# ittiam-systems/libxaac

Hardware: AMD Instinct MI355X
Metric: decoded audio frames/s (1024-spl IMDCT + complex QMF + HQ SBR + parametric stereo, HE-AACv2) (higher is better)
Workload: dtype int32

## Files before the change

### libxaac_amd/csrc/sbr_ps_frame.h

```cpp
#ifndef XAAC_SBR_PS_FRAME_H
#define XAAC_SBR_PS_FRAME_H

#include <stddef.h>

#include "sbr_ps.h"

#ifndef XP_T
#define XP_T(i)
#endif

#define XP_NO_PS_SCALE 0x7fffffff
#define XP_MAX_SEG (XAAC_PS_MAX_ENV + 2)

#if defined(__HIPCC__)
#define XP_UNROLL _Pragma("unroll")
#define XP_NOUNROLL _Pragma("nounroll")
#define XP_LAMBDA_INLINE __attribute__((always_inline))
#else
#define XP_UNROLL
#define XP_NOUNROLL
#define XP_LAMBDA_INLINE
#endif

struct XpFrameWork {
  union {
    int32_t hyb_u[3][2][44];
    uint32_t gscan[32][8];
    int32_t peak[32][20];
    uint32_t dl[32][13];
  };
  int32_t hyb_l[32][20];
  union {
    int32_t binpw[32][20];
    int16_t ratio[32][20];
  };
  uint32_t ap_h[32][11];
  uint32_t seg_hd[XP_MAX_SEG][4][24];
};
template <bool B>
struct XpBool {
  static constexpr bool value = B;
};

FX_HD int xp_popc(uint32_t v) { return __builtin_popcount(v); }
FX_HD int xp_clz(uint32_t v) { return __builtin_clz(v); }
FX_HD uint32_t xp_pack16(int16_t lo, int16_t hi) { return (uint32_t)(uint16_t)lo | ((uint32_t)(uint16_t)hi << 16); }
FX_HD int16_t xp_lo16(uint32_t v) { return (int16_t)(v & 0xffffu); }
FX_HD int16_t xp_hi16(uint32_t v) { return (int16_t)(v >> 16); }

FX_HD int32_t xp_dot2(uint32_t a, uint32_t b) {
#if defined(__HIP_DEVICE_COMPILE__)
  int32_t r;
  asm("v_dot2_i32_i16 %0, %1, %2, 0" : "=v"(r) : "v"(a), "v"(b));
  return r;
#else
  return (int32_t)((uint32_t)((int32_t)xp_lo16(a) * xp_lo16(b)) + (uint32_t)((int32_t)xp_hi16(a) * xp_hi16(b)));
#endif
}
FX_HD int16_t xp_seg_coeff(uint32_t hd, int n) { return (int16_t)(xp_hi16(hd) + n * xp_lo16(hd)); }
FX_HD uint32_t xp_load_pair(const int16_t *p) {
#if defined(__HIP_DEVICE_COMPILE__)
  typedef uint32_t __attribute__((may_alias)) xp_u32_alias;
  return *reinterpret_cast<const xp_u32_alias *>(p);
#else
  return xp_pack16(p[0], p[1]);
#endif
}
struct XpPhase {
  uint32_t re_pair, im_pair;
};
FX_HD XpPhase xp_phase_pairs(int16_t re, int16_t im) {
  XpPhase p;
  p.re_pair = xp_pack16(re, (int16_t)-im);
  p.im_pair = xp_pack16(im, re);
  return p;
}
FX_HD uint32_t xp_q15_pair(int32_t a, int32_t b) {
  return (((uint32_t)a >> 15) & 0xffffu) | (((uint32_t)b << 1) & 0xffff0000u);
}
FX_HD uint32_t xp_hi_pair(int32_t a, int32_t b) {
#if defined(__HIP_DEVICE_COMPILE__)
  return __builtin_amdgcn_perm((uint32_t)b, (uint32_t)a, 0x07060302u);
#else
  return ((uint32_t)a >> 16) | ((uint32_t)b & 0xffff0000u);
#endif
}
FX_HD uint32_t xp_mult16_shl_pair(uint32_t p, int32_t f2) {
#if defined(__HIP_DEVICE_COMPILE__)
  return xp_hi_pair(__mul24(xp_lo16(p), f2), __mul24(xp_hi16(p), f2));
#else
  return xp_hi_pair((int32_t)((uint32_t)(int32_t)xp_lo16(p) * (uint32_t)f2), (int32_t)((uint32_t)(int32_t)xp_hi16(p) * (uint32_t)f2));
#endif
}
FX_HD int32_t xp_m16x16_shl_pre(int16_t a, int32_t b2) {
#if defined(__HIP_DEVICE_COMPILE__)
  return __mul24(a, b2);
#else
  return (int32_t)((uint32_t)(int32_t)a * (uint32_t)b2);
#endif
}
FX_HD uint32_t xp_add16_pair(uint32_t a, uint32_t b) {
#if defined(__HIP_DEVICE_COMPILE__)
  typedef short xp_short2 __attribute__((ext_vector_type(2)));
  return __builtin_bit_cast(uint32_t, (xp_short2)(__builtin_bit_cast(xp_short2, a) + __builtin_bit_cast(xp_short2, b)));
#else
  return ((a + b) & 0xffffu) | ((a & 0xffff0000u) + (b & 0xffff0000u));
#endif
}
FX_HD uint32_t xp_sub16_pair(uint32_t a, uint32_t b) {
#if defined(__HIP_DEVICE_COMPILE__)
  typedef short xp_short2 __attribute__((ext_vector_type(2)));
  return __builtin_bit_cast(uint32_t, (xp_short2)(__builtin_bit_cast(xp_short2, a) - __builtin_bit_cast(xp_short2, b)));
#else
  return ((a - b) & 0xffffu) | ((a & 0xffff0000u) - (b & 0xffff0000u));
#endif
}
FX_HD uint32_t xp_allpass_packed(uint32_t &d0, uint32_t new_pair, const XpPhase &ph, uint32_t &e0, uint32_t &e1, uint32_t &e2,
                                 const XpPhase &p0, const XpPhase &p1, const XpPhase &p2, int16_t decay0, int16_t decay1,
                                 int16_t decay2) {
  uint32_t in = xp_q15_pair(xp_dot2(d0, ph.re_pair), xp_dot2(d0, ph.im_pair));
  d0 = new_pair;
  uint32_t *e[3] = {&e0, &e1, &e2};
  const XpPhase *pp[3] = {&p0, &p1, &p2};
  const int32_t decay2x[3] = {2 * decay0, 2 * decay1, 2 * decay2};
  XP_UNROLL
  for (int m = 0; m < 3; m++) {
    const uint32_t s = *e[m];
    const uint32_t t = xp_sub16_pair(xp_q15_pair(xp_dot2(s, pp[m]->re_pair), xp_dot2(s, pp[m]->im_pair)),
                                     xp_mult16_shl_pair(in, decay2x[m]));
    *e[m] = xp_add16_pair(in, xp_mult16_shl_pair(t, decay2x[m]));
    in = t;
  }
  return in;
}

FX_HD int32_t xp_adj_word(int32_t v, int shift) {
  if (shift > 31) shift = 31;
  if (shift < -31) shift = -31;
  const int shl = shift > 0 ? shift : 0, shr = shift < 0 ? -shift : 0;
  return (int32_t)((uint32_t)v << shl) >> shr;
}

FX_HD int32_t xp_bin_power_hyb(const XpTables *T, int bin, const int32_t *re, const int32_t *im) {
  if (bin < 2) {
    const int a = bin == 0 ? 0 : 4, b = bin == 0 ? 5 : 1;
    int32_t pw = xp_power(re[a], im[a]);
    pw = fx_add_sat(pw, fx_mul32x16(re[b], (int16_t)(re[b] >> 16)));
    return fx_add_sat(pw, fx_mul32x16(im[b], (int16_t)(im[b] >> 16)));
  }
  const int sb = T->borders_group[bin + 2];
  return xp_power(re[sb], im[sb]);
}

FX_HD uint32_t xp_gsum_addend(int32_t pw, int group_shift, bool counts) { return counts ? (uint32_t)(pw >> group_shift) : 0u; }
FX_HD uint32_t xp_gsum_scan(const XsCx &cx, uint32_t a, uint32_t &run) {
#if defined(__HIP_DEVICE_COMPILE__)
  int32_t r = (int32_t)a;
#define XP_DPP_ADD(ctrl, rows) r += __builtin_amdgcn_update_dpp(0, r, ctrl, rows, 0xf, false);
  XP_DPP_ADD(0x111, 0xf)
  XP_DPP_ADD(0x112, 0xf)
  XP_DPP_ADD(0x114, 0xf)
  XP_DPP_ADD(0x118, 0xf)
  XP_DPP_ADD(0x142, 0xa)
  XP_DPP_ADD(0x143, 0xc)
#undef XP_DPP_ADD
  (void)cx;
  (void)run;
  return (uint32_t)r;
#else
  (void)cx;
  run += a;
  return run;
#endif
}
FX_HD int32_t xp_gsum_sum(uint32_t s_last, uint32_t s_before) {
  const uint32_t d = s_last - s_before;
  return (int32_t)(d < 0x7fffffffu ? d : 0x7fffffffu);
}
FX_HD bool xp_gsum_fits(const XpTables *T) {
  if (T->borders_group[16] != 9) return false;
  for (int g = 0; g < 6; g++) {
    const int b0 = T->borders_group[16 + g], b1 = T->borders_group[17 + g], shift = T->group_shift[g];
    if (b1 <= b0 || b1 > 64 || shift < 0 || shift > 31) return false;
    if ((uint64_t)(b1 - b0) * (uint64_t)(0x7fffffff >> shift) >= ((uint64_t)1 << 32)) return false;
  }
  return true;
}

template <int NS = 32, class PS>
FX_HD int xp_ps_frame(const XsCx &cx, const XpTables *T, PS *ps, const xaac_ps_frame *pf, XpFrameWork *w, int32_t *xl,
                      int32_t *xr, int lb_scale, int ov_lb_scale, int hb_scale, int st_syn, int lsb, int usb,
                      int ps_scale_done = XP_NO_PS_SCALE) {
  static_assert(NS == 32 || NS == 30, "frames of 32 or 30 QMF slots");
#if defined(__HIP_DEVICE_COMPILE__)
  int32_t p1v[3][2], p3re[32], p3im[32];
  {
    const int l1 = cx.lane & 31;
    XP_UNROLL
    for (int b = 0; b < 3; b++) {
      p1v[b][0] = xl[(l1 + 6) * 128 + b];
      p1v[b][1] = xl[(l1 + 6) * 128 + 64 + b];
    }
    XP_UNROLL
    for (int l = 0; l < 32; l++) {
      p3re[l] = NS == 32 || l < NS ? xl[l * 128 + cx.lane] : 0;
      p3im[l] = NS == 32 || l < NS ? xl[l * 128 + 64 + cx.lane] : 0;
    }
  }
#endif
  const int ps_scale = ps_scale_done != XP_NO_PS_SCALE ? ps_scale_done : xp_init_ps_scale(cx, ps, lb_scale, ov_lb_scale, hb_scale);
  const int ov_lb_shift = ps_scale - ov_lb_scale, lb_shift = ps_scale - lb_scale, hb_shift = ps_scale - hb_scale;
  const int common_shift = (st_syn - ps_scale) - 8;
  XP_T(1);

  XS_PAR(l, 0, NS) {
    const int shiftdelay = l < NS - 6 ? 0 : (int16_t)(lb_scale - ps_scale);
    for (int b = 0; b < 3; b++) {
      const int sha = l + 6 < NS ? (b < lsb ? lb_shift : (b < usb ? hb_shift : 0)) : 0;
      for (int c = 0; c < 2; c++) {
#if defined(__HIP_DEVICE_COMPILE__)
        int32_t v = xp_adj_word(p1v[b][c], sha);
#else
        int32_t v = xp_adj_word(xl[(l + 6) * 128 + 64 * c + b], sha);
#endif
        v = shiftdelay < 0 ? fx_shl(v, -shiftdelay) : fx_shr(v, shiftdelay);
        w->hyb_u[b][c][12 + l] = v;
      }
    }
  }
  XS_PAR(i, 0, 12)
    for (int b = 0; b < 3; b++) {
      w->hyb_u[b][0][i] = ps->hyb_buf[b][0][i];
      w->hyb_u[b][1][i] = ps->hyb_buf[b][1][i];
    }
  cx.sync();
  XS_PAR(l, 0, NS) {
    int32_t re[8], im[8];
    xp_filt_8ch(T, &w->hyb_u[0][0][l], &w->hyb_u[0][1][l], re, im);
    for (int k = 0; k < 6; k++) {
      w->hyb_l[l][k] = re[k];
      w->hyb_l[l][10 + k] = im[k];
    }
  }
  XS_PAR(i, 0, 64) {
    const int b = 1 + (i >> 5), l = i & 31;
    if (NS != 32 && l >= NS) continue;
    int32_t re[2], im[2];
    xp_filt_2ch(T, &w->hyb_u[b][0][l], &w->hyb_u[b][1][l], re, im);
    w->hyb_l[l][4 + 2 * b] = re[0];
    w->hyb_l[l][5 + 2 * b] = re[1];
    w->hyb_l[l][14 + 2 * b] = im[0];
    w->hyb_l[l][15 + 2 * b] = im[1];
  }
  XS_PAR(i, 0, 12)
    for (int b = 0; b < 3; b++) {
      ps->hyb_buf[b][0][i] = w->hyb_u[b][0][NS + i];
      ps->hyb_buf[b][1][i] = w->hyb_u[b][1][NS + i];
    }
  cx.sync();
  XP_T(2);

  XS_PAR(g, 0, XAAC_PS_GROUPS) {
    w->seg_hd[0][0][g] = xp_pack16(ps->delta_h11_h12[2 * g], ps->H11_H12[2 * g]);
    w->seg_hd[0][1][g] = xp_pack16(ps->delta_h11_h12[2 * g + 1], ps->H11_H12[2 * g + 1]);
    w->seg_hd[0][2][g] = xp_pack16(ps->delta_h21_h22[2 * g], ps->H21_H22[2 * g]);
    w->seg_hd[0][3][g] = xp_pack16(ps->delta_h21_h22[2 * g + 1], ps->H21_H22[2 * g + 1]);
  }
  const int usb_prev = cx.uni(ps->usb);
  uint32_t seg_mask = 0;
  int clear_slot = NS;
  {
    int env = 0, nseg = 1;
    int next = cx.uni(pf->border_position[0]);
    for (int l = 0; l < NS; l++) {
      if (l == next) {
        if (env == 0) clear_slot = l;
        cx.sync();
        xp_rot_env_coeffs(cx, T, ps, pf, env);
        XS_PAR(g, 0, XAAC_PS_GROUPS) {
          w->seg_hd[nseg][0][g] = xp_pack16(ps->delta_h11_h12[2 * g], ps->H11_H12[2 * g]);
          w->seg_hd[nseg][1][g] = xp_pack16(ps->delta_h11_h12[2 * g + 1], ps->H11_H12[2 * g + 1]);
          w->seg_hd[nseg][2][g] = xp_pack16(ps->delta_h21_h22[2 * g], ps->H21_H22[2 * g]);
          w->seg_hd[nseg][3][g] = xp_pack16(ps->delta_h21_h22[2 * g + 1], ps->H21_H22[2 * g + 1]);
        }
        seg_mask |= 1u << l;
        nseg++;
        env++;
        next = env <= XAAC_PS_MAX_ENV ? cx.uni(pf->border_position[env]) : 64;
      }
    }
  }
  cx.sync();
  XP_T(3);

  {
    XP_UNROLL
    for (int c = 0; c < 4; c++) {
      uint32_t run[8] = {0, 0, 0, 0, 0, 0, 0, 0};
      XS_PAR(sb, 0, 64) {
        int32_t rre[8], rim[8];
        XP_UNROLL
        for (int ls = 0; ls < 8; ls++) {
#if defined(__HIP_DEVICE_COMPILE__)
          rre[ls] = p3re[8 * c + ls];
          rim[ls] = p3im[8 * c + ls];
#else
          rre[ls] = xl[(8 * c + ls) * 128 + sb];
          rim[ls] = xl[(8 * c + ls) * 128 + 64 + sb];
#endif
        }
        const int gsh = sb < 11 ? 0 : (sb < 18 ? 1 : (sb < 23 ? 2 : (sb < 35 ? 3 : 4)));
        const bool own_bin = sb >= 3 && sb < 9;
        int gcol = 6;
        XP_UNROLL
        for (int g = 0; g < 6; g++) gcol = sb == T->borders_group[17 + g] - 1 ? g : gcol;
        int32_t *dst = own_bin ? &w->binpw[8 * c][sb + 5] : reinterpret_cast<int32_t *>(&w->gscan[8 * c][gcol]);
        const int dstride = own_bin ? 20 : 8;
        XP_UNROLL
        for (int ls = 0; ls < 8; ls++) {
          const int l = 8 * c + ls;
          const int usb_l = l >= clear_slot ? usb : usb_prev;
          const int sh = sb < lsb ? (l < 6 ? ov_lb_shift : lb_shift) : (sb < usb ? hb_shift : 0);
          const int32_t re = xp_adj_word(rre[ls], sh), im = xp_adj_word(rim[ls], sh);
          const int32_t pw = xp_power(re, im);
          const uint32_t s = xp_gsum_scan(cx, xp_gsum_addend(pw, gsh, sb >= 9 && sb < usb_l), run[ls]);
          dst[ls * dstride] = own_bin ? pw : (int32_t)s;
        }
      }
    }
  }
  cx.sync();
  XS_PAR(i, 0, 6 * NS) {
    const int l = i / 6, g = i % 6;
    const uint32_t prev = w->gscan[l][g > 0 ? g - 1 : 0];
    const uint32_t before = g > 0 ? prev : 0u;
    w->binpw[l][14 + g] = xp_gsum_sum(w->gscan[l][g], before);
  }
  XS_PAR(i, 0, 8 * NS) {
    const int l = i >> 3, bin = i & 7;
    w->binpw[l][bin] = xp_bin_power_hyb(T, bin, &w->hyb_l[l][0], &w->hyb_l[l][10]);
  }
  cx.sync();
  XP_T(4);

  XS_PAR(bin, 0, 20) {
    int32_t pd = ps->peak_decay_diff[bin], pdp = ps->peak_decay_diff_prev[bin], nrg = ps->energy_prev[bin];
    int32_t pin[NS];
    XP_UNROLL
    for (int l = 0; l < NS; l++) pin[l] = w->binpw[l][bin];
    XP_UNROLL
    for (int l = 0; l < NS; l++) {
      int32_t pw = fx_shl(pin[l], 1);
      if (pw < 0) pw = 0;
      pd = fx_mul32x16_shl(pd, 0x620a);
      if (pw > pd) pd = pw;
      pdp = fx_add_sat(fx_mul32x16_shl(pdp, 0x6000), fx_sub_sat(pd, pw) >> 2);
      nrg = fx_add_sat(fx_mul32x16_shl(nrg, 0x6000), pw >> 2);
      w->binpw[l][bin] = nrg;
      w->peak[l][bin] = fx_add_sat(pdp, pdp >> 1);
    }
    ps->peak_decay_diff[bin] = pd;
    ps->peak_decay_diff_prev[bin] = pdp;
    ps->energy_prev[bin] = nrg;
  }
  cx.sync();
  for (int i0 = 0; i0 < 20 * NS; i0 += 64) {
    int16_t q = 0;
    XS_PAR(i, i0, (20 * NS) % 64 == 0 || i0 + 64 < 20 * NS ? i0 + 64 : 20 * NS) {
      const int32_t pk = (&w->peak[0][0])[i], nrg = (&w->binpw[0][0])[i];
      q = pk <= nrg ? (int16_t)0x7fff : (int16_t)xp_divide16_pos(nrg, pk);
#if !defined(__HIP_DEVICE_COMPILE__)
      (&w->ratio[0][0])[i] = q;
#endif
    }
#if defined(__HIP_DEVICE_COMPILE__)
    cx.sync();
    (&w->ratio[0][0])[i0 + cx.lane] = q;
    cx.sync();
#endif
  }
  cx.sync();
  XP_T(5);

  {
    const int idx0 = cx.uni(ps->idx), idx_long0 = cx.uni(ps->idx_long);
    const int is0 = cx.uni(ps->idx_ser[0]), is1 = cx.uni(ps->idx_ser[1]), is2 = cx.uni(ps->idx_ser[2]);
    const int clear_lo = (usb > usb_prev && usb_prev) ? usb_prev : 64;
    const int clear_hi = usb < 23 ? usb : 23;
    const int p14_0 = idx_long0 % 14;
    const int cs_right = common_shift < 0 ? (-common_shift > 31 ? 31 : -common_shift) : 0;
    uint32_t events = seg_mask | (1u << 6) | (1u << 14);
    if (clear_slot < NS) events |= 1u << clear_slot;
    if (clear_slot + 14 < NS) events |= 1u << (clear_slot + 14);
    XS_PAR(sb, 0, 64) {
      const int qmf_chain = sb >= 3 && sb < 23, hyb_chain = sb >= 32 && sb < 42, chain = qmf_chain || hyb_chain;
      const int csb = qmf_chain ? sb : (hyb_chain ? sb - 32 : 3);
      const int di = 9 + 3 * (csb - 3);
      const int16_t *ph = hyb_chain ? &T->frac_delay_phase_fac_qmf_sub_re_im[2 * csb] : &T->frac_delay_phase_fac_qmf_re_im[2 * csb];
      const int16_t *pser = hyb_chain ? &T->frac_delay_phase_fac_qmf_sub_ser_re_im[2 * csb] : &T->frac_delay_phase_fac_qmf_ser_re_im[2 * csb];
      const int pstep = hyb_chain ? 32 : 64;
      const XpPhase phase = xp_phase_pairs(ph[0], ph[1]);
      const XpPhase ps0 = xp_phase_pairs(pser[0], pser[1]), ps1 = xp_phase_pairs(pser[pstep], pser[pstep + 1]),
                    ps2 = xp_phase_pairs(pser[2 * pstep], pser[2 * pstep + 1]);
      const int16_t dec0 = hyb_chain ? T->rev_link_decay_ser[0] : T->decay_scale_factor[qmf_chain ? di : 9];
      const int16_t dec1 = hyb_chain ? T->rev_link_decay_ser[1] : T->decay_scale_factor[qmf_chain ? di + 1 : 10];
      const int16_t dec2 = hyb_chain ? T->rev_link_decay_ser[2] : T->decay_scale_factor[qmf_chain ? di + 2 : 11];
      uint32_t d0[2] = {0, 0}, r0[3] = {0, 0, 0}, r1[4] = {0, 0, 0, 0}, r2[5] = {0, 0, 0, 0, 0};
      if (chain) {
        XP_UNROLL
        for (int j = 0; j < 2; j++) {
          const int16_t *q = hyb_chain ? &ps->sub[(idx0 + j) % 2][2 * csb] : &ps->ap[(idx0 + j) % 2][2 * csb];
          d0[j] = xp_pack16(q[0], q[1]);
        }
        XP_UNROLL
        for (int j = 0; j < 3; j++) {
          const int16_t *q = hyb_chain ? &ps->sub_ser[(is0 + j) % 3][0][2 * csb] : &ps->ser[(is0 + j) % 3][0][2 * csb];
          r0[j] = xp_pack16(q[0], q[1]);
        }
        XP_UNROLL
        for (int j = 0; j < 4; j++) {
          const int16_t *q = hyb_chain ? &ps->sub_ser[(is1 + j) % 4][1][2 * csb] : &ps->ser[(is1 + j) % 4][1][2 * csb];
          r1[j] = xp_pack16(q[0], q[1]);
        }
        XP_UNROLL
        for (int j = 0; j < 5; j++) {
          const int16_t *q = hyb_chain ? &ps->sub_ser[(is2 + j) % 5][2][2 * csb] : &ps->ser[(is2 + j) % 5][2][2 * csb];
          r2[j] = xp_pack16(q[0], q[1]);
        }
      }
      const int g = T->band_to_group[sb];
      const int bin_sb = sb < 23 ? T->delay_to_bin[sb] : (sb < 35 ? 18 : 19);
      uint32_t h11, h12, h21, h22, d11, d12, d21, d22;
      const auto seg_load = [&](int s) {
        const uint32_t a = w->seg_hd[s][0][g], b = w->seg_hd[s][1][g], c = w->seg_hd[s][2][g], d = w->seg_hd[s][3][g];
        h11 = a & 0xffff0000u, h12 = b & 0xffff0000u, h21 = c & 0xffff0000u, h22 = d & 0xffff0000u;
        d11 = a << 16, d12 = b << 16, d21 = c << 16, d22 = d << 16;
      };
      seg_load(0);
      uint32_t prev = sb >= 35 ? xp_pack16(ps->sd[2 * (sb - 35)], ps->sd[2 * (sb - 35) + 1]) : 0u;
      const int is_ap = sb < 23, is_d14 = sb >= 23 && sb < 35;
      int shl_ov, shr_ov, shl_lb, shr_lb;
      {
        const int s_ov = sb < lsb ? ov_lb_shift : (sb < usb ? hb_shift : 0), s_lb = sb < lsb ? lb_shift : (sb < usb ? hb_shift : 0);
        const int c_ov = s_ov > 31 ? 31 : (s_ov < -31 ? -31 : s_ov), c_lb = s_lb > 31 ? 31 : (s_lb < -31 ? -31 : s_lb);
        shl_ov = c_ov > 0 ? c_ov : 0, shr_ov = c_ov < 0 ? -c_ov : 0;
        shl_lb = c_lb > 0 ? c_lb : 0, shr_lb = c_lb < 0 ? -c_lb : 0;
      }
      int shl = shl_ov, shr = shr_ov;
      bool active = sb < usb_prev, fed14 = false;
      const int ldj = is_d14 ? 2 * (sb - 23) : 0, dlj = is_d14 ? sb - 23 : 12, apj = hyb_chain ? csb : 10;
      int ld_at = 24 * p14_0;
      const int16_t *const ld_lane = &ps->ld[0][ldj];
      static_assert(sizeof(ps->ld[0]) == 24 * sizeof(int16_t), "rows of the 14-slot ring: 24 int16, whole words");
      static_assert(offsetof(PS, ld) % 4 == 0 && alignof(PS) % 4 == 0, "the 14-slot ring starts on a word of a word-aligned state");
      int16_t tr_nx = w->ratio[0][bin_sb];
      int32_t hre_nx = w->hyb_l[0][csb], him_nx = w->hyb_l[0][10 + csb];
      uint32_t ld_nx = xp_load_pair(ld_lane + ld_at);
      int32_t nre[4], nim[4];
      XP_UNROLL
      for (int j = 0; j < 4; j++) {
        nre[j] = xl[j * 128 + sb];
        nim[j] = xl[j * 128 + 64 + sb];
      }
      const auto walk = [&](auto cs_positive) XP_LAMBDA_INLINE {
        XP_NOUNROLL
        for (int l0 = 0; l0 < NS; l0 += 4) {
          int32_t cre[4], cim[4];
          XP_UNROLL
          for (int j = 0; j < 4; j++) {
            cre[j] = nre[j];
            cim[j] = nim[j];
          }
          if (l0 + 4 < NS) {
            XP_UNROLL
            for (int j = 0; j < 4; j++) {
              nre[j] = xl[(l0 + 4 + j) * 128 + sb];
              nim[j] = xl[(l0 + 4 + j) * 128 + 64 + sb];
            }
          }
          const uint32_t events4 = events >> l0;
          XP_UNROLL
          for (int j = 0; j < 4; j++) {
            const int l = l0 + j;
            if (NS % 4 != 0 && l >= NS) break;
            const int16_t tr = tr_nx;
            const int32_t hre = hre_nx, him = him_nx;
            const uint32_t ld_cur = ld_nx;
            {
              const int ln = l + 1 < NS ? l + 1 : NS - 1;
              ld_at = ld_at + 24 == 14 * 24 ? 0 : ld_at + 24;
              tr_nx = w->ratio[ln][bin_sb];
              hre_nx = w->hyb_l[ln][csb];
              him_nx = w->hyb_l[ln][10 + csb];
              ld_nx = xp_load_pair(ld_lane + ld_at);
            }
            if ((events4 >> j) & 1u) {
#if defined(__HIP_DEVICE_COMPILE__)
              asm volatile("");
#endif
              shl = l < 6 ? shl_ov : shl_lb;
              shr = l < 6 ? shr_ov : shr_lb;
              active = sb < (l >= clear_slot ? usb : usb_prev);
              fed14 = l >= 14 && sb < (l - 14 >= clear_slot ? usb : usb_prev);
              if (l == clear_slot) {
                const int c = qmf_chain && sb >= clear_lo && sb < clear_hi;
                XP_UNROLL
                for (int m = 0; m < 3; m++) r0[m] = c ? 0u : r0[m];
                XP_UNROLL
                for (int m = 0; m < 4; m++) r1[m] = c ? 0u : r1[m];
                XP_UNROLL
                for (int m = 0; m < 5; m++) r2[m] = c ? 0u : r2[m];
              }
              if ((seg_mask >> l) & 1u)
                seg_load(xp_popc(seg_mask & (0xffffffffu >> (31 - l))));
            }
            const int32_t re0 = (int32_t)((uint32_t)cre[j] << shl) >> shr, im0 = (int32_t)((uint32_t)cim[j] << shl) >> shr;
            const int16_t q_re = fx_round16(re0), q_im = fx_round16(im0);
            const uint32_t q = xp_pack16(q_re, q_im);
            const uint32_t in_pair = hyb_chain ? xp_pack16(fx_round16(hre), fx_round16(him)) : q;
            uint32_t dv = d0[0], e0 = r0[0], e1 = r1[0], e2 = r2[0];
            const uint32_t o_chain = xp_allpass_packed(dv, in_pair, phase, e0, e1, e2, ps0, ps1, ps2, dec0, dec1, dec2);
            d0[0] = d0[1];
            d0[1] = dv;
            r0[0] = r0[1]; r0[1] = r0[2];
            r0[2] = e0;
            r1[0] = r1[1]; r1[1] = r1[2]; r1[2] = r1[3];
            r1[3] = e1;
            r2[0] = r2[1]; r2[1] = r2[2]; r2[2] = r2[3]; r2[3] = r2[4];
            r2[4] = e2;
            w->ap_h[l][apj] = o_chain;
            h11 += d11;
            h12 += d12;
            h21 += d21;
            h22 += d22;
            const uint32_t o14_new = w->dl[l >= 14 ? l - 14 : 0][dlj];
            const uint32_t o14 = fed14 ? o14_new : ld_cur;
            const uint32_t o = is_ap ? o_chain : (is_d14 ? o14 : prev);
            w->dl[l][dlj] = q;
            prev = active ? q : prev;
            int32_t re = re0, im = im0;
            int32_t r_re = xp_m16x16_shl_pre(xp_lo16(o), 2 * tr), r_im = xp_m16x16_shl_pre(xp_hi16(o), 2 * tr);
            xp_rotate_w(&re, &r_re, h11, h12, h21, h22);
            xp_rotate_w(&im, &r_im, h11, h12, h21, h22);
            re = active ? re : re0;
            im = active ? im : im0;
            r_re = active ? r_re : 0;
            r_im = active ? r_im : 0;
            if (decltype(cs_positive)::value) {
              re = fx_shl_sat(re, common_shift);
              im = fx_shl_sat(im, common_shift);
            } else {
              re = re >> cs_right;
              im = im >> cs_right;
            }
            if (sb >= 3) {
              xl[l * 128 + sb] = re;
              xl[l * 128 + 64 + sb] = im;
              xr[l * 128 + sb] = r_re;
              xr[l * 128 + 64 + sb] = r_im;
            }
          }
        }
      };
      if (common_shift > 0)
        walk(XpBool<true>());
      else
        walk(XpBool<false>());
      if (chain) {
        XP_UNROLL
        for (int j = 0; j < 2; j++) {
          int16_t *q = hyb_chain ? &ps->sub[(idx0 + j) % 2][2 * csb] : &ps->ap[(idx0 + j) % 2][2 * csb];
          q[0] = xp_lo16(d0[j]);
          q[1] = xp_hi16(d0[j]);
        }
        XP_UNROLL
        for (int j = 0; j < 3; j++) {
          int16_t *q = hyb_chain ? &ps->sub_ser[(is0 + NS + j) % 3][0][2 * csb] : &ps->ser[(is0 + NS + j) % 3][0][2 * csb];
          q[0] = xp_lo16(r0[j]);
          q[1] = xp_hi16(r0[j]);
        }
        XP_UNROLL
        for (int j = 0; j < 4; j++) {
          int16_t *q = hyb_chain ? &ps->sub_ser[(is1 + NS + j) % 4][1][2 * csb] : &ps->ser[(is1 + NS + j) % 4][1][2 * csb];
          q[0] = xp_lo16(r1[j]);
          q[1] = xp_hi16(r1[j]);
        }
        XP_UNROLL
        for (int j = 0; j < 5; j++) {
          int16_t *q = hyb_chain ? &ps->sub_ser[(is2 + NS + j) % 5][2][2 * csb] : &ps->ser[(is2 + NS + j) % 5][2][2 * csb];
          q[0] = xp_lo16(r2[j]);
          q[1] = xp_hi16(r2[j]);
        }
      }
      if (sb >= 35) {
        ps->sd[2 * (sb - 35)] = xp_lo16(prev);
        ps->sd[2 * (sb - 35) + 1] = xp_hi16(prev);
      }
      if (is_d14) {
        for (int l = (clear_slot == 0 || usb == usb_prev) ? NS - 14 : 0; l < NS; l++) {
          const int pos = (idx_long0 + l) % 14;
          if (sb < (l >= clear_slot ? usb : usb_prev)) {
            ps->ld[pos][ldj] = xp_lo16(w->dl[l][dlj]);
            ps->ld[pos][ldj + 1] = xp_hi16(w->dl[l][dlj]);
          }
        }
      }
    }
    cx.sync();
    XS_ONE {
      ps->idx = (int16_t)idx0;
      ps->idx_ser[0] = (int16_t)((is0 + NS) % 3);
      ps->idx_ser[1] = (int16_t)((is1 + NS) % 4);
      ps->idx_ser[2] = (int16_t)((is2 + NS) % 5);
      ps->idx_long = (int16_t)((idx_long0 + NS) % 14);
      if (clear_slot < NS) ps->usb = (int16_t)usb;
    }
  }
  cx.sync();
  XP_T(6);

  XS_PAR(i, 0, 2 * NS) {
    const int l = i >> 1, c = i & 1;
    const uint32_t below = seg_mask & (0xffffffffu >> (31 - l));
    const int s = xp_popc(below), nn = l - (below ? 31 - xp_clz(below) : 0) + 1;
    int32_t acc_l[3] = {0, 0, 0}, acc_r[3] = {0, 0, 0};
    XP_UNROLL
    for (int sb = 0; sb < 10; sb++) {
      const int b = sb < 6 ? 0 : (sb < 8 ? 1 : 2);
      const bool first = sb == 0 || sb == 6 || sb == 8;
      const int16_t h11 = xp_seg_coeff(w->seg_hd[s][0][sb], nn), h12 = xp_seg_coeff(w->seg_hd[s][1][sb], nn);
      const int16_t h21 = xp_seg_coeff(w->seg_hd[s][2][sb], nn), h22 = xp_seg_coeff(w->seg_hd[s][3][sb], nn);
      const int16_t tr = w->ratio[l][T->hybrid_to_bin[sb]];
      const uint32_t o = w->ap_h[l][sb];
      int32_t lv = w->hyb_l[l][10 * c + sb];
      int32_t rv = xp_m16x16_shl(c ? xp_hi16(o) : xp_lo16(o), tr);
      xp_rotate(&lv, &rv, h11, h12, h21, h22);
      acc_l[b] = first ? lv : fx_add_sat(acc_l[b], lv);
      acc_r[b] = first ? rv : fx_add_sat(acc_r[b], rv);
    }
    XP_UNROLL
    for (int b = 0; b < 3; b++) {
      int32_t v = acc_l[b];
      if (common_shift < 0)
        v = fx_shr(v, -common_shift > 31 ? 31 : -common_shift);
      else if (common_shift > 0)
        v = fx_shl_sat(v, common_shift);
      xl[l * 128 + 64 * c + b] = v;
      xr[l * 128 + 64 * c + b] = acc_r[b];
    }
  }
  {
    const int s = xp_popc(seg_mask), n = NS - (seg_mask ? 31 - xp_clz(seg_mask) : 0);
    XS_PAR(g, 0, XAAC_PS_GROUPS) {
      ps->H11_H12[2 * g] = xp_seg_coeff(w->seg_hd[s][0][g], n);
      ps->H11_H12[2 * g + 1] = xp_seg_coeff(w->seg_hd[s][1][g], n);
      ps->H21_H22[2 * g] = xp_seg_coeff(w->seg_hd[s][2][g], n);
      ps->H21_H22[2 * g + 1] = xp_seg_coeff(w->seg_hd[s][3][g], n);
    }
  }
  cx.sync();
  XP_T(7);
  return ps_scale;
}

#endif
```

### libxaac_amd/csrc/sbr_ps_kernel.hip

```cpp
#include <hip/hip_runtime.h>
#include <stddef.h>
#include <stdint.h>
#include <stdlib.h>

#ifdef XS_PROFILE
__shared__ long long xp_prof_last;
__shared__ long long xp_prof_acc[16];
#define XP_T(i)                                   \
  do {                                            \
    if (threadIdx.x == 0) {                       \
      long long t_ = clock64();                   \
      xp_prof_acc[i] += t_ - xp_prof_last;        \
      xp_prof_last = t_;                          \
    }                                             \
  } while (0)
#else
#define XP_T(i)
#endif
#define XS_SYNC_WAVE_LDS 1
#include "sbr_ps_frame.h"
#include "sbr_ps_kernel.h"

namespace {

struct XpLdsState {
  XAAC_PS_STATE_HEAD_FIELDS
};
constexpr int kHeadWords = offsetof(xaac_ps_state, syn_ring_r) / 4;
static_assert(offsetof(xaac_ps_state, syn_ring_r) % 4 == 0 && sizeof(XpLdsState) == kHeadWords * 4, "mirror layout");
static_assert(sizeof(xaac_ps_frame) % 4 == 0, "word copies");

constexpr int kTabBytes = (int)sizeof(XpTables);
#ifndef XP_WAVES
#define XP_WAVES 4
#endif
#ifndef XP_WAVES_PER_EU
#define XP_WAVES_PER_EU 2
#endif
constexpr int kPsWaves = XP_WAVES;
struct XpLds {
  XpLdsState ps;
  xaac_ps_frame pf;
  XpFrameWork w;
};

__device__ __forceinline__ void xp_wave_sync() {
  __builtin_amdgcn_fence(__ATOMIC_RELEASE, "wavefront");
  __builtin_amdgcn_wave_barrier();
  __builtin_amdgcn_fence(__ATOMIC_ACQUIRE, "wavefront");
}

__device__ __forceinline__ void copy_words(int32_t *dst, const int32_t *src, int n, int lane) {
  for (int i = lane; i < n; i += 64 * 8) {
    int32_t t[8];
#pragma unroll
    for (int j = 0; j < 8; j++)
      if (i + 64 * j < n) t[j] = src[i + 64 * j];
#pragma unroll
    for (int j = 0; j < 8; j++)
      if (i + 64 * j < n) dst[i + 64 * j] = t[j];
  }
}

template <int NS>
__device__ __forceinline__ int xp_init_ps_scale_regs(const XsCx &cx, int32_t (&rs)[NS], int lb_scale, int ov_lb_scale, int hb_scale) {
  constexpr int W_AP = offsetof(XpLdsState, ap) / 4, W_LD = offsetof(XpLdsState, ld) / 4, W_SD = offsetof(XpLdsState, sd) / 4;
  constexpr int W_SUB = offsetof(XpLdsState, sub) / 4, W_IDX = offsetof(XpLdsState, idx_ser) / 4;
  constexpr int W_PK = offsetof(XpLdsState, peak_decay_diff) / 4, W_HYB = offsetof(XpLdsState, hyb_buf) / 4;
  constexpr int W_H = offsetof(XpLdsState, h11_h12_vec) / 4, W_DBS = offsetof(XpLdsState, delay_buffer_scale) / 4;
  static_assert(offsetof(XpLdsState, ser) == 0 && W_AP == 480 && W_LD == W_AP + 64 && W_SD == W_LD + 168 && W_SUB == W_SD + 32, "layout");
  static_assert(W_IDX == W_SUB + 32 + 240 && offsetof(XpLdsState, sample_ser) == 4 * W_IDX + 6 && W_PK == W_IDX + 4, "layout");
  static_assert(W_HYB == W_PK + 60 && W_H == W_HYB + 72 && offsetof(XpLdsState, delay_buffer_scale) % 4 == 0 && W_DBS < 64 * NS, "layout");
  const auto word_of = [&](int w) { return __builtin_amdgcn_readlane(rs[w / 64], w % 64); };
  const int ss0 = word_of(W_IDX + 1) >> 16, ss1 = (int16_t)word_of(W_IDX + 2), ss2 = word_of(W_IDX + 2) >> 16;
  const auto is_pair = [&](int w) -> bool {
    const int k = w & 31, blk = w >> 5;
    const bool mid = k >= 3 && k <= 22;
    if (w < W_AP) {
      const int i = blk % 3, j = blk / 3;
      return mid && j < (i == 0 ? ss0 : (i == 1 ? ss1 : ss2));
    }
    if (w < W_LD) return mid;
    if (w < W_SD + 29) return true;
    if (w < W_SUB) return false;
    return w < W_IDX;
  };
  int32_t m16 = 0, m32 = 0;
#pragma unroll
  for (int j = 0; j < NS; j++) {
    const int w = cx.lane + 64 * j;
    const int32_t v = rs[j], lo = (int16_t)v, hi = v >> 16;
    m16 |= is_pair(w) ? (fx_abs_nrm(lo) | fx_abs_nrm(hi)) : 0;
    if (64 * j + 63 >= W_HYB && 64 * j < W_H) m32 |= (w >= W_HYB && w < W_H) ? fx_abs_nrm(v) : 0;
  }
  const int reserve = xs_pnorm32(cx.wave_or((int32_t)((uint32_t)m16 << 16) | m32));
  const int dbs = (int16_t)((int16_t)word_of(W_DBS) + reserve);
  int16_t t = (int16_t)(lb_scale < ov_lb_scale ? lb_scale : ov_lb_scale);
  if (hb_scale < t) t = (int16_t)hb_scale;
  if (dbs < t) t = (int16_t)dbs;
  const int ps_scale = t - 1;
  const int scale = (int16_t)((ps_scale - dbs) + reserve);
  if (scale != 0) {
    const int l16 = scale > 0 ? (scale > 15 ? 15 : scale) : 0, r16 = scale < 0 ? (-scale > 31 ? 31 : -scale) : 0;
#pragma unroll
    for (int j = 0; j < NS; j++) {
      const int w = cx.lane + 64 * j;
      const int32_t v = rs[j];
      if (64 * j < W_IDX) {
        const int32_t lo = (int16_t)v, hi = v >> 16;
        const int16_t a = fx_sat16(xs_shl(lo, l16) >> r16), b = fx_sat16(xs_shl(hi, l16) >> r16);
        rs[j] = is_pair(w) ? (int32_t)xp_pack16(a, b) : v;
      }
      if (64 * j + 63 >= W_PK && 64 * j < W_H) {
        const bool pk = w >= W_PK && w < W_HYB, hy = w >= W_HYB && w < W_H;
        const int sc = pk ? 2 * scale : scale;
        const int32_t r = sc > 0 ? fx_shl_sat(rs[j], sc) : fx_shr(rs[j], -sc);
        rs[j] = (pk || hy) ? r : rs[j];
      }
    }
  }
  if (cx.lane == W_DBS % 64) rs[W_DBS / 64] = (int32_t)((uint32_t)rs[W_DBS / 64] & 0xffff0000u) | (uint16_t)(int16_t)ps_scale;
  return ps_scale;
}

template <int NF, int NSL = 32>
__device__ __forceinline__ int xp_frame_sanitize_regs(const XsCx &cx, int32_t (&rf)[NF]) {
  constexpr int E_BORDER = offsetof(xaac_ps_frame, border_position) / 2, E_IID = offsetof(xaac_ps_frame, iid_par_table) / 2;
  constexpr int E_ICC = offsetof(xaac_ps_frame, icc_par_table) / 2, E_END = sizeof(xaac_ps_frame) / 2;
  static_assert(offsetof(xaac_ps_frame, iid_quant) == 0 && E_BORDER + XAAC_PS_MAX_ENV + 2 < E_IID && E_IID % 2 == 0 && E_ICC % 2 == 0, "layout");
  const int steps = (int16_t)__builtin_amdgcn_readlane(rf[0], 0) ? 15 : 7;
  int bad = 0;
#pragma unroll
  for (int j = 0; j < NF; j++) {
    const int w = cx.lane + 64 * j;
    const int32_t v = rf[j];
    int h[2] = {(int16_t)v, v >> 16};
#pragma unroll
    for (int c = 0; c < 2; c++) {
      const int e = 2 * w + c;
      const bool border = e >= E_BORDER && e < E_BORDER + XAAC_PS_MAX_ENV + 2, iid = e >= E_IID && e < E_ICC, icc = e >= E_ICC && e < E_END;
      const int lo = border ? 0 : (iid ? -steps : (icc ? 0 : -32768)), hi = border ? NSL : (iid ? steps : (icc ? 7 : 32767));
      const int t = h[c] < lo ? lo : (h[c] > hi ? hi : h[c]);
      bad |= t != h[c];
      h[c] = t;
    }
    rf[j] = (int32_t)xp_pack16((int16_t)h[0], (int16_t)h[1]);
  }
  return cx.wave_or(bad) != 0;
}

}

template <int NSL = 32>
__global__ __launch_bounds__(64 * kPsWaves, XP_WAVES_PER_EU) void xaac_ps_kernel(XaacPsParams p) {
  __shared__ XpLds sw[kPsWaves];
  __shared__ int32_t s_tabs[(kTabBytes + 3) / 4];
  const int lane = threadIdx.x & 63, wave = __builtin_amdgcn_readfirstlane(threadIdx.x >> 6);
  XpLds &s = sw[wave];
  const XsCx cx = {lane, 64};
  for (int i = threadIdx.x; i < (kTabBytes + 3) / 4; i += 64 * kPsWaves) s_tabs[i] = reinterpret_cast<const int32_t *>(&xaac_ps_tables)[i];
  __syncthreads();
  const XpTables *tabs = reinterpret_cast<const XpTables *>(s_tabs);
#ifdef XP_STAGGER_G
  if (p.n >= 3 * (int)gridDim.x * kPsWaves)
    for (int t = 0; t < ((int)blockIdx.x * kPsWaves + wave) % XP_STAGGER_G; t++) __builtin_amdgcn_s_sleep(XP_STAGGER_SLEEP);
#endif
#ifdef XS_PROFILE
  if (threadIdx.x == 0) {
    for (int i = 0; i < 16; i++) xp_prof_acc[i] = 0;
  }
#endif
  for (int n = blockIdx.x * kPsWaves + wave; n < p.n; n += gridDim.x * kPsWaves) {
    xaac_ps_state *gps = p.state + n;
    int32_t *gx = p.x + (size_t)n * (40 * 128) + 2 * 128;
    int32_t *gr = p.xr + (size_t)n * (32 * 128);
    int16_t *par = p.par_l + 8 * (size_t)n;
    constexpr int NS = (kHeadWords + 63) / 64, NF = (sizeof(xaac_ps_frame) / 4 + 63) / 64;
    int32_t rs[NS], rf[NF];
    const int32_t *gs = reinterpret_cast<const int32_t *>(gps), *gf = reinterpret_cast<const int32_t *>(p.frame + n);
    const int apply_v = p.sbr_frame[n].apply_processing, mode_v = p.header[n].channel_mode;
    const int par_v = lane < (NSL != 32 ? 8 : 6) ? par[lane] : 0;
    const int tail_v = lane < 3 ? (lane == 0 ? gps->st_syn_scale_r : (lane == 1 ? gps->syn_lsb_r : gps->syn_usb_r)) : 0;

#pragma unroll
    for (int j = 0; j < NS; j++) rs[j] = lane + 64 * j < kHeadWords ? gs[lane + 64 * j] : 0;
#pragma unroll
    for (int j = 0; j < NF; j++) rf[j] = lane + 64 * j < (int)(sizeof(xaac_ps_frame) / 4) ? gf[lane + 64 * j] : 0;
    if (NSL != 32 && __builtin_amdgcn_readlane(par_v, 7)) {
      if (lane == 0) p.par_r[8 * (size_t)n + 6] = 1;
      continue;
    }
    if (!(__builtin_amdgcn_readfirstlane(apply_v) && __builtin_amdgcn_readfirstlane(mode_v) == 3)) {
      if (lane == 0) {
        p.par_l[8 * (size_t)n + 6] = 0;
        p.par_r[8 * (size_t)n + 6] = 1;
      }
      continue;
    }
    const int lb_scale = __builtin_amdgcn_readlane(par_v, 0), ov_lb_scale = __builtin_amdgcn_readlane(par_v, 1);
    const int hb_scale = __builtin_amdgcn_readlane(par_v, 2), st_syn = __builtin_amdgcn_readlane(par_v, 3);
    const int lsb = __builtin_amdgcn_readlane(par_v, 4), usb = __builtin_amdgcn_readlane(par_v, 5);
    const int ps_scale_done = xp_init_ps_scale_regs<NS>(cx, rs, lb_scale, ov_lb_scale, hb_scale);
    const int ps_clamped = xp_frame_sanitize_regs<NF, NSL>(cx, rf);
    xp_wave_sync();
#pragma unroll
    for (int j = 0; j < NS; j++)
      if (lane + 64 * j < kHeadWords) reinterpret_cast<int32_t *>(&s.ps)[lane + 64 * j] = rs[j];
#pragma unroll
    for (int j = 0; j < NF; j++)
      if (lane + 64 * j < (int)(sizeof(xaac_ps_frame) / 4)) reinterpret_cast<int32_t *>(&s.pf)[lane + 64 * j] = rf[j];
    xp_wave_sync();
#ifdef XS_PROFILE
    if (threadIdx.x == 0) xp_prof_last = clock64();
#endif
    const int ps_scale =
        xp_ps_frame<NSL>(cx, tabs, &s.ps, &s.pf, &s.w, gx, gr, lb_scale, ov_lb_scale, hb_scale, st_syn, lsb, usb, ps_scale_done);
    xp_wave_sync();
    {
      int32_t *dst = reinterpret_cast<int32_t *>(gps);
      const int32_t *src = reinterpret_cast<const int32_t *>(&s.ps);
      for (int i = lane; i < kHeadWords; i += 64) dst[i] = src[i];
    }
    if (lane == 0) {
      int16_t *pr = p.par_r + 8 * (size_t)n;
      const int16_t ready = (int16_t)(st_syn - 8);
      par[0] = par[1] = par[2] = ready;
      pr[0] = pr[1] = pr[2] = (int16_t)ps_scale;
      pr[3] = (int16_t)__builtin_amdgcn_readlane(tail_v, 0);
      pr[4] = (int16_t)__builtin_amdgcn_readlane(tail_v, 1);
      pr[5] = (int16_t)__builtin_amdgcn_readlane(tail_v, 2);
      pr[6] = 0;
      par[6] = 0;
      gps->lb_scale_r = gps->ov_lb_scale_r = gps->hb_scale_r = (int16_t)ps_scale;
      p.sbr_state[n].ps_scale = (int16_t)ps_scale;
#ifndef XS_PROFILE
      if (ps_clamped && p.status) p.status[n] = -1;
#endif
    }
  }
#ifdef XS_PROFILE
  __syncthreads();
  if (threadIdx.x < 16 && p.dbg) atomicAdd(reinterpret_cast<unsigned long long *>(p.dbg) + 32 + lane, (unsigned long long)xp_prof_acc[lane]);
#endif
}

__global__ __launch_bounds__(64) void xaac_sbr_handover_kernel(xaac_sbr_handover_batch b) {
  const int e = blockIdx.x, lane = threadIdx.x;
  const xaac_sbr_state *src = b.state + b.src[e];
  if (b.mode == XAAC_HANDOVER_PS_START) {
    xaac_ps_state *dst = b.ps_state + b.dst[e];
    for (int i = lane; i < 1280; i += 64) dst->syn_ring_r[i] = src->syn_ring[i];
    if (lane == 0) dst->st_syn_scale_r = src->st_syn_scale;
  } else {
    xaac_sbr_state *dst = b.state + b.dst[e];
    for (int i = lane; i < 1280; i += 64) dst->syn_ring[i] = src->syn_ring[i];
    for (int i = lane; i < 320; i += 64) dst->ana_ring[i] = src->ana_ring[i];
    for (int i = lane; i < 6 * 64; i += 64) dst->overlap[i] = src->overlap[i];
    if (lane == 0) {
      dst->st_syn_scale = src->st_syn_scale;
      dst->st_lb_scale = src->st_lb_scale;
      dst->ov_lb_scale = src->ov_lb_scale;
      dst->ov_hb_scale = src->ov_hb_scale;
    }
  }
}

__global__ __launch_bounds__(256) void xaac_sbr_apply_side_kernel(xaac_sbr_apply_side_batch b) {
  const int e = blockIdx.x * 256 + threadIdx.x;
  if (e >= b.n_streams * b.ch_fac) return;
  const int i = e / b.ch_fac, c = e % b.ch_fac;
  const int32_t *f = b.flags + 8 * (size_t)i;
  const int reset = f[1], reset_channels = f[2], upsampling = f[3];
  if (!reset && !upsampling) return;
  xaac_sbr_state *s = b.state + e;
  const xaac_sbr_header *h = b.header + (size_t)i * b.ch_fac;
  if (reset && c < reset_channels) {
    s->ph_index = 0;
    s->filt_buf_noise_e = 0;
    s->start_up = 1;
    s->syn_lsb = s->codec_usb = h->sub_band_start;
    s->syn_usb = h->sub_band_end;
    for (int k = 0; k < XAAC_SBR_MAX_PATCHES; k++) s->bw_array_prev[k] = 0;
  }
  if (upsampling) {
    s->syn_lsb = s->codec_usb = 32;
    s->syn_usb = 64;
  }
  if (b.ps_state && c == 0) {
    xaac_ps_state *ps = b.ps_state + i;
    if (reset && reset_channels > 1) {
      ps->syn_lsb_r = h->sub_band_start;
      ps->syn_usb_r = h->sub_band_end;
    }
    if (upsampling) {
      ps->syn_lsb_r = 32;
      ps->syn_usb_r = 64;
    }
  }
}

extern "C" hipError_t xaac_launch_sbr_apply_side(const xaac_sbr_apply_side_batch *b, hipStream_t stream) {
  const int n = b->n_streams * b->ch_fac;
  hipLaunchKernelGGL(xaac_sbr_apply_side_kernel, dim3((n + 255) / 256), dim3(256), 0, stream, *b);
  return hipGetLastError();
}

extern "C" hipError_t xaac_launch_sbr_handover(const xaac_sbr_handover_batch *b, hipStream_t stream) {
  hipLaunchKernelGGL(xaac_sbr_handover_kernel, dim3(b->n), dim3(64), 0, stream, *b);
  return hipGetLastError();
}

extern "C" hipError_t xaac_launch_ps(const XaacPsParams *p, hipStream_t stream) {
  static int resident = 0;
  if (!resident) {
    int per_cu = 0, dev = 0;
    hipDeviceProp_t prop;
    if (hipOccupancyMaxActiveBlocksPerMultiprocessor(&per_cu, xaac_ps_kernel<32>, 64 * kPsWaves, 0) != hipSuccess || per_cu < 1) per_cu = 2;
    if (hipGetDevice(&dev) != hipSuccess || hipGetDeviceProperties(&prop, dev) != hipSuccess) prop.multiProcessorCount = 256;
    const char *e = getenv("XAAC_PS_WG_PER_CU");
    if (e && atoi(e) > 0) per_cu = atoi(e);
    resident = per_cu * (prop.multiProcessorCount > 0 ? prop.multiProcessorCount : 256);
  }
  const int need = (p->n + kPsWaves - 1) / kPsWaves, grid = need < resident ? need : resident;
  if (p->n_slots == 30)
    hipLaunchKernelGGL(xaac_ps_kernel<30>, dim3(grid), dim3(64 * kPsWaves), 0, stream, *p);
  else
    hipLaunchKernelGGL(xaac_ps_kernel<32>, dim3(grid), dim3(64 * kPsWaves), 0, stream, *p);
  return hipGetLastError();
}

extern "C" hipError_t xaac_warm_sbr_ps(void) {
  hipFuncAttributes a;
  return hipFuncGetAttributes(&a, reinterpret_cast<const void *>(&xaac_ps_kernel<32>));
}
```

Baseline: 17.89 million.

## Parallelize transient smoothing, use rcp-based division, unroll 14-slot delay ring

Splits the per-bin transient peak/energy recursion into 40 lanes (peak and energy chains run on separate lanes) instead of 20. Replaces the per-element divide with a float-reciprocal quotient plus a single remainder correction, applied over all 64 lanes. Stages the 14-slot long delay ring into LDS scratch before the decorrelation loop and writes it back in a bulk, word-wide pass afterwards. This removes the fed14 bookkeeping and the per-sb serial write-back loop. It also hoists shift selection out of the group-sum loop and adds asm phase markers for inspection. The risks are bit-exactness of the reciprocal divide and extra LDS traffic and syncs.

```diff
diff --git a/libxaac_amd/csrc/sbr_ps_frame.h b/libxaac_amd/csrc/sbr_ps_frame.h
--- a/libxaac_amd/csrc/sbr_ps_frame.h
+++ b/libxaac_amd/csrc/sbr_ps_frame.h
@@ -27,7 +27,7 @@
     int32_t hyb_u[3][2][44];
     uint32_t gscan[32][8];
     int32_t peak[32][20];
-    uint32_t dl[32][13];
+    uint32_t dl[14 + 32][13];
   };
   int32_t hyb_l[32][20];
   union {
@@ -37,6 +37,7 @@
   uint32_t ap_h[32][11];
   uint32_t seg_hd[XP_MAX_SEG][4][24];
 };
+static_assert(sizeof(XpFrameWork::dl) <= sizeof(XpFrameWork::peak), "the unrolled 14-slot lines fit the scratch union as it was");
 template <bool B>
 struct XpBool {
   static constexpr bool value = B;
@@ -64,6 +65,15 @@
   return *reinterpret_cast<const xp_u32_alias *>(p);
 #else
   return xp_pack16(p[0], p[1]);
+#endif
+}
+FX_HD void xp_store_pair(int16_t *p, uint32_t v) {
+#if defined(__HIP_DEVICE_COMPILE__)
+  typedef uint32_t __attribute__((may_alias)) xp_u32_alias;
+  *reinterpret_cast<xp_u32_alias *>(p) = v;
+#else
+  p[0] = xp_lo16(v);
+  p[1] = xp_hi16(v);
 #endif
 }
 struct XpPhase {
@@ -141,6 +151,31 @@
   return (int32_t)((uint32_t)v << shl) >> shr;
 }
 
+FX_HD uint32_t xp_quot15_rcp(uint32_t u, uint32_t v, float r) {
+  const uint32_t n = u << 15;
+  uint32_t q = (uint32_t)((float)n * r);
+#if defined(__HIP_DEVICE_COMPILE__)
+  const int32_t rem = (int32_t)(n - __umul24(q, v));
+#else
+  const int32_t rem = (int32_t)(n - q * v);
+#endif
+  q += rem >= (int32_t)v ? 1u : 0u;
+  q -= rem < 0 ? 1u : 0u;
+  return q;
+}
+FX_HD uint32_t xp_quot15(uint32_t u, uint32_t v) {
+#if defined(__HIP_DEVICE_COMPILE__)
+  return xp_quot15_rcp(u, v, __builtin_amdgcn_rcpf((float)v));
+#else
+  return xp_quot15_rcp(u, v, 1.0f / (float)v);
+#endif
+}
+FX_HD int32_t xp_divide16_norm(int32_t op1, int32_t op2) {
+  const int nrm = fx_norm32(op2);
+  const uint32_t u = (uint32_t)xs_shl(op1, nrm) >> 16, v = (uint32_t)xs_shl(op2, nrm) >> 16;
+  return (int32_t)(xp_quot15(u, v) & 0xffffu);
+}
+
 FX_HD int32_t xp_bin_power_hyb(const XpTables *T, int bin, const int32_t *re, const int32_t *im) {
   if (bin < 2) {
     const int a = bin == 0 ? 0 : 4, b = bin == 0 ? 5 : 1;
@@ -153,6 +188,8 @@
 }
 
 FX_HD uint32_t xp_gsum_addend(int32_t pw, int group_shift, bool counts) { return counts ? (uint32_t)(pw >> group_shift) : 0u; }
+FX_HD int xp_gsum_shift(int group_shift, bool counts) { return counts ? group_shift : 31; }
+FX_HD uint32_t xp_gsum_addend_sh(int32_t pw, int shift) { return (uint32_t)(pw >> shift); }
 FX_HD uint32_t xp_gsum_scan(const XsCx &cx, uint32_t a, uint32_t &run) {
 #if defined(__HIP_DEVICE_COMPILE__)
   int32_t r = (int32_t)a;
@@ -185,6 +222,57 @@
     if ((uint64_t)(b1 - b0) * (uint64_t)(0x7fffffff >> shift) >= ((uint64_t)1 << 32)) return false;
   }
   return true;
+}
+
+template <int NS, class PS>
+FX_HD void xp_transient_frame(const XsCx &cx, PS *ps, XpFrameWork *w) {
+  XS_PAR(i, 0, 32 + 20) {
+    const int bin = i & 31;
+    const bool en = i >= 32;
+    if (bin >= 20) continue;
+    int32_t pd = ps->peak_decay_diff[bin], acc = en ? ps->energy_prev[bin] : ps->peak_decay_diff_prev[bin];
+    int32_t *out = en ? &w->binpw[0][bin] : &w->peak[0][bin];
+    int32_t pin[NS];
+    XP_UNROLL
+    for (int l = 0; l < NS; l++) pin[l] = w->binpw[l][bin];
+    cx.sync();
+    XP_UNROLL
+    for (int l = 0; l < NS; l++) {
+      int32_t pw = fx_shl(pin[l], 1);
+      if (pw < 0) pw = 0;
+      pd = fx_mul32x16_shl(pd, 0x620a);
+      if (pw > pd) pd = pw;
+      const int32_t t = en ? pw : fx_sub_sat(pd, pw);
+      acc = fx_add_sat(fx_mul32x16_shl(acc, 0x6000), t >> 2);
+      out[20 * l] = en ? acc : fx_add_sat(acc, acc >> 1);
+    }
+    if (en) {
+      ps->energy_prev[bin] = acc;
+    } else {
+      ps->peak_decay_diff[bin] = pd;
+      ps->peak_decay_diff_prev[bin] = acc;
+    }
+  }
+  cx.sync();
+#if defined(__HIP_DEVICE_COMPILE__)
+  {
+    int32_t pk[10], nrg[10];
+    XP_UNROLL
+    for (int t = 0; t < 10; t++) {
+      pk[t] = (&w->peak[0][0])[64 * t + cx.lane];
+      nrg[t] = (&w->binpw[0][0])[64 * t + cx.lane];
+    }
+    cx.sync();
+    XP_UNROLL
+    for (int t = 0; t < 10; t++)
+      (&w->ratio[0][0])[64 * t + cx.lane] = pk[t] <= nrg[t] ? (int16_t)0x7fff : (int16_t)xp_divide16_norm(nrg[t], pk[t]);
+  }
+#else
+  for (int i = 0; i < 20 * NS; i++) {
+    const int32_t pk = (&w->peak[0][0])[i], nrg = (&w->binpw[0][0])[i];
+    (&w->ratio[0][0])[i] = pk <= nrg ? (int16_t)0x7fff : (int16_t)xp_divide16_norm(nrg, pk);
+  }
+#endif
 }
 
 template <int NS = 32, class PS>
@@ -316,14 +404,15 @@
         for (int g = 0; g < 6; g++) gcol = sb == T->borders_group[17 + g] - 1 ? g : gcol;
         int32_t *dst = own_bin ? &w->binpw[8 * c][sb + 5] : reinterpret_cast<int32_t *>(&w->gscan[8 * c][gcol]);
         const int dstride = own_bin ? 20 : 8;
+        const int sh_ov = sb < lsb ? ov_lb_shift : (sb < usb ? hb_shift : 0), sh_lb = sb < lsb ? lb_shift : (sb < usb ? hb_shift : 0);
+        const int gsh_old = xp_gsum_shift(gsh, sb >= 9 && sb < usb_prev), gsh_new = xp_gsum_shift(gsh, sb >= 9 && sb < usb);
         XP_UNROLL
         for (int ls = 0; ls < 8; ls++) {
           const int l = 8 * c + ls;
-          const int usb_l = l >= clear_slot ? usb : usb_prev;
-          const int sh = sb < lsb ? (l < 6 ? ov_lb_shift : lb_shift) : (sb < usb ? hb_shift : 0);
+          const int sh = l < 6 ? sh_ov : sh_lb;
           const int32_t re = xp_adj_word(rre[ls], sh), im = xp_adj_word(rim[ls], sh);
           const int32_t pw = xp_power(re, im);
-          const uint32_t s = xp_gsum_scan(cx, xp_gsum_addend(pw, gsh, sb >= 9 && sb < usb_l), run[ls]);
+          const uint32_t s = xp_gsum_scan(cx, xp_gsum_addend_sh(pw, l >= clear_slot ? gsh_new : gsh_old), run[ls]);
           dst[ls * dstride] = own_bin ? pw : (int32_t)s;
         }
       }
@@ -343,42 +432,7 @@
   cx.sync();
   XP_T(4);
 
-  XS_PAR(bin, 0, 20) {
-    int32_t pd = ps->peak_decay_diff[bin], pdp = ps->peak_decay_diff_prev[bin], nrg = ps->energy_prev[bin];
-    int32_t pin[NS];
-    XP_UNROLL
-    for (int l = 0; l < NS; l++) pin[l] = w->binpw[l][bin];
-    XP_UNROLL
-    for (int l = 0; l < NS; l++) {
-      int32_t pw = fx_shl(pin[l], 1);
-      if (pw < 0) pw = 0;
-      pd = fx_mul32x16_shl(pd, 0x620a);
-      if (pw > pd) pd = pw;
-      pdp = fx_add_sat(fx_mul32x16_shl(pdp, 0x6000), fx_sub_sat(pd, pw) >> 2);
-      nrg = fx_add_sat(fx_mul32x16_shl(nrg, 0x6000), pw >> 2);
-      w->binpw[l][bin] = nrg;
-      w->peak[l][bin] = fx_add_sat(pdp, pdp >> 1);
-    }
-    ps->peak_decay_diff[bin] = pd;
-    ps->peak_decay_diff_prev[bin] = pdp;
-    ps->energy_prev[bin] = nrg;
-  }
-  cx.sync();
-  for (int i0 = 0; i0 < 20 * NS; i0 += 64) {
-    int16_t q = 0;
-    XS_PAR(i, i0, (20 * NS) % 64 == 0 || i0 + 64 < 20 * NS ? i0 + 64 : 20 * NS) {
-      const int32_t pk = (&w->peak[0][0])[i], nrg = (&w->binpw[0][0])[i];
-      q = pk <= nrg ? (int16_t)0x7fff : (int16_t)xp_divide16_pos(nrg, pk);
-#if !defined(__HIP_DEVICE_COMPILE__)
-      (&w->ratio[0][0])[i] = q;
-#endif
-    }
-#if defined(__HIP_DEVICE_COMPILE__)
-    cx.sync();
-    (&w->ratio[0][0])[i0 + cx.lane] = q;
-    cx.sync();
-#endif
-  }
+  xp_transient_frame<NS>(cx, ps, w);
   cx.sync();
   XP_T(5);
 
@@ -389,9 +443,17 @@
     const int clear_hi = usb < 23 ? usb : 23;
     const int p14_0 = idx_long0 % 14;
     const int cs_right = common_shift < 0 ? (-common_shift > 31 ? 31 : -common_shift) : 0;
-    uint32_t events = seg_mask | (1u << 6) | (1u << 14);
+    uint32_t events = seg_mask | (1u << 6);
     if (clear_slot < NS) events |= 1u << clear_slot;
-    if (clear_slot + 14 < NS) events |= 1u << (clear_slot + 14);
+    static_assert(sizeof(ps->ld[0]) == 24 * sizeof(int16_t), "rows of the 14-slot ring: 24 int16, whole words");
+    static_assert(offsetof(PS, ld) % 4 == 0 && alignof(PS) % 4 == 0, "the 14-slot ring starts on a word of a word-aligned state");
+    XS_PAR(i, 0, 4 * 14) {
+      const int r = i >> 2, j0 = 3 * (i & 3);
+      const int pos = p14_0 + r >= 14 ? p14_0 + r - 14 : p14_0 + r;
+      XP_UNROLL
+      for (int k = 0; k < 3; k++) w->dl[r][j0 + k] = xp_load_pair(&ps->ld[pos][2 * (j0 + k)]);
+    }
+    cx.sync();
     XS_PAR(sb, 0, 64) {
       const int qmf_chain = sb >= 3 && sb < 23, hyb_chain = sb >= 32 && sb < 42, chain = qmf_chain || hyb_chain;
       const int csb = qmf_chain ? sb : (hyb_chain ? sb - 32 : 3);
@@ -447,15 +509,11 @@
         shl_lb = c_lb > 0 ? c_lb : 0, shr_lb = c_lb < 0 ? -c_lb : 0;
       }
       int shl = shl_ov, shr = shr_ov;
-      bool active = sb < usb_prev, fed14 = false;
-      const int ldj = is_d14 ? 2 * (sb - 23) : 0, dlj = is_d14 ? sb - 23 : 12, apj = hyb_chain ? csb : 10;
-      int ld_at = 24 * p14_0;
-      const int16_t *const ld_lane = &ps->ld[0][ldj];
-      static_assert(sizeof(ps->ld[0]) == 24 * sizeof(int16_t), "rows of the 14-slot ring: 24 int16, whole words");
-      static_assert(offsetof(PS, ld) % 4 == 0 && alignof(PS) % 4 == 0, "the 14-slot ring starts on a word of a word-aligned state");
+      bool active = sb < usb_prev;
+      const int dlj = is_d14 ? sb - 23 : 12, apj = hyb_chain ? csb : 10;
       int16_t tr_nx = w->ratio[0][bin_sb];
       int32_t hre_nx = w->hyb_l[0][csb], him_nx = w->hyb_l[0][10 + csb];
-      uint32_t ld_nx = xp_load_pair(ld_lane + ld_at);
+      uint32_t o14_nx = w->dl[0][dlj];
       int32_t nre[4], nim[4];
       XP_UNROLL
       for (int j = 0; j < 4; j++) {
@@ -485,14 +543,13 @@
             if (NS % 4 != 0 && l >= NS) break;
             const int16_t tr = tr_nx;
             const int32_t hre = hre_nx, him = him_nx;
-            const uint32_t ld_cur = ld_nx;
+            const uint32_t o14 = o14_nx;
             {
               const int ln = l + 1 < NS ? l + 1 : NS - 1;
-              ld_at = ld_at + 24 == 14 * 24 ? 0 : ld_at + 24;
               tr_nx = w->ratio[ln][bin_sb];
               hre_nx = w->hyb_l[ln][csb];
               him_nx = w->hyb_l[ln][10 + csb];
-              ld_nx = xp_load_pair(ld_lane + ld_at);
+              o14_nx = w->dl[l + 1][dlj];
             }
             if ((events4 >> j) & 1u) {
 #if defined(__HIP_DEVICE_COMPILE__)
@@ -501,7 +558,6 @@
               shl = l < 6 ? shl_ov : shl_lb;
               shr = l < 6 ? shr_ov : shr_lb;
               active = sb < (l >= clear_slot ? usb : usb_prev);
-              fed14 = l >= 14 && sb < (l - 14 >= clear_slot ? usb : usb_prev);
               if (l == clear_slot) {
                 const int c = qmf_chain && sb >= clear_lo && sb < clear_hi;
                 XP_UNROLL
@@ -533,11 +589,10 @@
             h12 += d12;
             h21 += d21;
             h22 += d22;
-            const uint32_t o14_new = w->dl[l >= 14 ? l - 14 : 0][dlj];
-            const uint32_t o14 = fed14 ? o14_new : ld_cur;
-            const uint32_t o = is_ap ? o_chain : (is_d14 ? o14 : prev);
-            w->dl[l][dlj] = q;
-            prev = active ? q : prev;
+            const uint32_t held = is_d14 ? o14 : prev;
+            const uint32_t o = is_ap ? o_chain : held;
+            prev = active ? q : held;
+            w->dl[l + 14][dlj] = prev;
             int32_t re = re0, im = im0;
             int32_t r_re = xp_m16x16_shl_pre(xp_lo16(o), 2 * tr), r_im = xp_m16x16_shl_pre(xp_hi16(o), 2 * tr);
             xp_rotate_w(&re, &r_re, h11, h12, h21, h22);
@@ -596,17 +651,14 @@
         ps->sd[2 * (sb - 35)] = xp_lo16(prev);
         ps->sd[2 * (sb - 35) + 1] = xp_hi16(prev);
       }
-      if (is_d14) {
-        for (int l = (clear_slot == 0 || usb == usb_prev) ? NS - 14 : 0; l < NS; l++) {
-          const int pos = (idx_long0 + l) % 14;
-          if (sb < (l >= clear_slot ? usb : usb_prev)) {
-            ps->ld[pos][ldj] = xp_lo16(w->dl[l][dlj]);
-            ps->ld[pos][ldj + 1] = xp_hi16(w->dl[l][dlj]);
-          }
-        }
-      }
     }
     cx.sync();
+    XS_PAR(i, 0, 4 * 14) {
+      const int r = i >> 2, j0 = 3 * (i & 3), p0 = (idx_long0 + NS) % 14;
+      const int pos = p0 + r >= 14 ? p0 + r - 14 : p0 + r;
+      XP_UNROLL
+      for (int k = 0; k < 3; k++) xp_store_pair(&ps->ld[pos][2 * (j0 + k)], w->dl[NS + r][j0 + k]);
+    }
     XS_ONE {
       ps->idx = (int16_t)idx0;
       ps->idx_ser[0] = (int16_t)((is0 + NS) % 3);
diff --git a/libxaac_amd/csrc/sbr_ps_kernel.hip b/libxaac_amd/csrc/sbr_ps_kernel.hip
--- a/libxaac_amd/csrc/sbr_ps_kernel.hip
+++ b/libxaac_amd/csrc/sbr_ps_kernel.hip
@@ -14,6 +14,8 @@
       xp_prof_last = t_;                          \
     }                                             \
   } while (0)
+#elif defined(XP_PHASE_MARKS)
+#define XP_T(i) asm volatile("; XP_PHASE " #i)
 #else
 #define XP_T(i)
 #endif
@@ -212,6 +214,8 @@
     xp_wave_sync();
 #ifdef XS_PROFILE
     if (threadIdx.x == 0) xp_prof_last = clock64();
+#elif defined(XP_PHASE_MARKS)
+    XP_T(0);
 #endif
     const int ps_scale =
         xp_ps_frame<NSL>(cx, tabs, &s.ps, &s.pf, &s.w, gx, gr, lb_scale, ov_lb_scale, hb_scale, st_syn, lsb, usb, ps_scale_done);
```

Result: faster. 18.33 million (median of 6 runs) (+2.5%).
